# mrazomej/BarBay.jl

Measured on AMD Instinct MI355X. Metric: ELBO-grad steps/sec, 50k barcodes x 8 timepoints, higher is better.
Workload: dtype f64

## Files before the change

barbay.jl_amd/csrc/bb_engine.hip:

```cpp
#include "../../include/barbay_hip.h"
#include "bb_block.h"
#include "bb_persist.h"
#include "bb_resident.h"
#include "bb_stream.h"
#include "bb_inst.h"
#include "bb_hier.h"
#include "bb_ppc.h"
#include "bb_freq.h"
#include "bb_score.h"
#include "bb_rb.h"
#include "bb_chain.h"
#include "bb_trace.h"
#include "bb_logp.h"
#include "bb_mathprobe.h"

#include <algorithm>
#include <cmath>
#include <cstdarg>
#include <cstdio>
#include <cstdlib>
#include <cstring>
#include <ctime>
#include <string>
#include <type_traits>
// ... 228 lines not shown
            bbp_prefetch_slot<KIND, PP>(cx, h->M, h->S, A, h->NB, st + (size_t)b * h->nthr, bb_slot_of(A, step).slot);
            bbp_residual_ahead<KIND>(cx, h->M, h->NB, A);
            if (xg) bbp_consume<true>(cx, h->M, h->S, A, L, par, epoch, &E.ok, abs_epoch);
            else bbp_consume<false>(cx, h->M, h->S, A, L, par, epoch, &E.ok, abs_epoch);
            bbp_finish<KIND>(cx, h->M, h->S, A, h->NB);
            bbp_update<KIND, PP>(cx, h->M, h->S, A, h->NB, st + (size_t)b * h->nthr, bb_slot_of(A, step));
        }
    } else {
        for (int b = 0; b < h->nblk; ++b) {
            BBCtx cx = cxof(b);
            bbp_epilogue<KIND, PP>(cx, h->M, h->S, A, h->NB, st + (size_t)b * h->nthr, (unsigned long long)(h->step + nsteps), E.ok == 0);
        }
    }
}

template <int KIND, int PP, bool AP, bool OS = false>
static void emu_res_phase(EmuPersist& E, int phase, long long it, long long nsteps) {
    bb_handle* h = E.h;
    const RunArgs& A = E.A;
    BRSt<PP>* st = (BRSt<PP>*)E.st.data();
    auto cxof = [&](int b) { return BBCtx{h->nthr, b, E.lds.data() + (size_t)b * (h->lds_doubles_p + 64), nullptr}; };
    const BRLay& Y = h->Yh;
    const int NS = A.S < 1 ? 1 : A.S;
    const bool MSrun = NS > 1 || A.elbo_every > 0;
    const unsigned long long step = (unsigned long long)(h->step + it / NS);
    const int smp = (int)(it % NS);
    const bool last = smp == NS - 1;
    const unsigned long long xc = MSrun ? step * (unsigned long long)NS + (unsigned long long)smp : step;
    const int buf = (int)(xc & 1);
    const bool want_el = MSrun && A.elbo_every > 0 && step % (unsigned long long)A.elbo_every == 0;
    const int ring = A.elbo_every > 0 ? (int)((step / (unsigned long long)A.elbo_every) % BB_ELBO_RING) : 0;
    const bool xg = h->p2p_on;
    const BBSlot wslot = bb_slot_of(A, step);
    for (int b = 0; b < (phase == 2 ? bbp_groups(A) : h->plan.nblk); ++b) {
        BBCtx cx = cxof(b);
        BRSt<PP>* sb = st + (size_t)b * h->nthr;
        if (phase == 0) {
            br_prologue<KIND, PP, AP>(cx, h->M, h->S, A, Y, h->plan.NB, sb);
            br_draw_ahead<KIND, PP, AP>(cx, A, Y, sb, (unsigned long long)h->step);
        } else if (phase == 1) {
            if (MSrun) br_sample<KIND, PP, true>(cx, h->M, h->S, A, Y, sb, buf, wslot.slot, last, want_el);
            else br_sample<KIND, PP, false, false, OS>(cx, h->M, h->S, A, Y, sb, buf, wslot.slot);
            const unsigned epoch = A.xepoch0 + (unsigned)(xc + 1);
            if (MSrun) br_moments<KIND, PP, true>(cx, h->M, h->S, Y, sb, buf, epoch, want_el);
            else br_moments<KIND, PP, false>(cx, h->M, h->S, Y, sb, buf, epoch);
            br_xchg_publish<KIND, PP, AP, false, OS>(cx, h->M, h->S, A, Y, sb, xc, wslot.slot, last ? step + 1 : step, last ? 0u : (unsigned)(smp + 1), last);
        } else if (phase == 2) {
            if (xg) br_xchg_lead<true>(cx, h->M, h->S, A, Y, xc, &E.ok);
            else br_xchg_lead<false>(cx, h->M, h->S, A, Y, xc, &E.ok);
        } else if (phase == 3) {
            if (xg && MSrun) br_xchg_consume<KIND, PP, true, true>(cx, h->M, h->S, A, Y, sb, xc, &E.ok, want_el, ring, smp);
            else if (xg) br_xchg_consume<KIND, PP, true, false>(cx, h->M, h->S, A, Y, sb, xc, &E.ok);
            else if (MSrun) br_xchg_consume<KIND, PP, false, true>(cx, h->M, h->S, A, Y, sb, xc, &E.ok, want_el, ring, smp);
            else br_xchg_consume<KIND, PP, false, false>(cx, h->M, h->S, A, Y, sb, xc, &E.ok);
            if (MSrun) br_update<KIND, PP, 0, AP, true>(cx, h->M, h->S, A, Y, sb, wslot, buf, h->plan.NB, smp, NS);
            else if (!AP && uniform_T(h->M) == 8) br_update<KIND, PP, 8, false, false, false, OS>(cx, h->M, h->S, A, Y, sb, wslot, buf, h->plan.NB);
            else if (!AP && uniform_T(h->M) == 6) br_update<KIND, PP, 6, false, false, false, OS>(cx, h->M, h->S, A, Y, sb, wslot, buf, h->plan.NB);
            else br_update<KIND, PP, 0, AP, false, false, OS>(cx, h->M, h->S, A, Y, sb, wslot, buf, h->plan.NB);
        } else {
            br_epilogue<KIND, PP, AP>(cx, h->S, sb, (unsigned long long)(h->step + nsteps), E.ok == 0);
        }
    }
}

template <int KIND, int TT, bool MS, bool OS = false>
static void emu_stream_phase(EmuPersist& E, int phase, long long it, long long nsteps) {
    bb_handle* h = E.h;
    const RunArgs& A = E.A;
    BSG* gs = (BSG*)E.st.data();
    auto cxof = [&](int b) { return BBCtx{h->nthr, b, E.lds.data() + (size_t)b * (h->lds_doubles_p + 64), nullptr}; };
    const BRLay& Y = h->Yh;
    const int NS = MS ? (A.S < 1 ? 1 : A.S) : 1;
    const unsigned long long step = (unsigned long long)(h->step + it / NS);
    const int smp = (int)(it % NS);
    const unsigned long long xc = step * (unsigned long long)NS + (unsigned long long)smp;
    auto rec = [&](unsigned long long st_) { return MS && A.elbo_every > 0 && st_ % (unsigned long long)A.elbo_every == 0; };
    const bool want_el = rec(step);
    const int ring = A.elbo_every > 0 ? (int)((step / (unsigned long long)A.elbo_every) % BB_ELBO_RING) : 0;
    const BSMs ms = MS ? bs_ms_of(A, step, smp, NS, want_el, rec(step + 1)) : bs_ms_plain((unsigned)step);
    BRSt<1>* nost = nullptr;
    for (int b = 0; b < (phase == 2 ? bbp_groups(A) : h->plan.nblk); ++b) {
        BBCtx cx = cxof(b);
        BSG* gb = gs + (size_t)b * h->nthr;
        int* bad_any = (int*)(cx.lds + Y.L.misc) + 3;
        if (phase == 0) {
            br_tile_setup<KIND>(cx, h->M, h->S, A, Y, h->plan.NB, KIND <= 2 ? h->nthr / 16 : h->nthr / 64);
            *bad_any = 0;
            bs_sample0<KIND, TT, MS>(cx, h->M, h->S, A, Y, h->plan.NB, h->plan.P, (unsigned)h->step, gb, (int)(((unsigned long long)h->step * (unsigned long long)NS) & 1ull), rec((unsigned long long)h->step));
        } else if (phase == 1) {
            bs_moments<KIND, TT, MS>(cx, h->M, h->S, A, Y, h->plan.NB, h->plan.P, (unsigned)step, gb, ms.buf, want_el);
            br_row_publish<1, MS>(cx, h->M, h->S, Y, nost, A.xepoch0 + (unsigned)(xc + 1), want_el);
        } else if (phase == 2) {
            br_xchg_lead<false>(cx, h->M, h->S, A, Y, xc, &E.ok);
        } else if (phase == 3) {
            br_xchg_consume<KIND, 1, false, MS>(cx, h->M, h->S, A, Y, nost, xc, &E.ok, want_el, ring, smp);
            bs_update_l<KIND, TT, MS, OS>(cx, h->M, h->S, A, Y, h->plan.NB, h->plan.P, (unsigned)step, bb_slot_of(A, step), bad_any, gb, ms);
            bs_update_u<KIND, TT, MS, OS>(cx, h->M, h->S, A, Y, h->plan.NB, h->plan.P, (unsigned)step, bb_slot_of(A, step), bad_any, gb, ms);
        } else {
            if (*bad_any) h->S.hstatus[1] = 1u;
            if (b == 0) { h->S.ctr[0] = (unsigned long long)(h->step + nsteps); h->S.ctr[1] = h->S.ctr[0]; }
        }
    }
}

static void emu_persist_dispatch(EmuPersist& E, int phase, long long it, long long nsteps) {
    const LaunchPlan& p = E.h->plan;
// ... 621 lines not shown
```

barbay.jl_amd/csrc/bb_persist.h:

```cpp
#pragma once
#include "bb_block.h"
#include <string.h>

template <int KIND>
BB_DEV BBLds bbp_layout(const BBCtx& cx, const DevModel& M, int NB) {
    if (cx.lay) return *(const BBLds*)cx.lay;
    return bb_lds_layout(M.R, M.E, KIND, M.Ttot, M.nt1, M.K, NB, cx.nthr, 1);
}

template <int P>
struct BBPst {
    bb_d2 mu[P], om[P], am[P], ao[P];
    bb_d2 a[P], h[P];
    bb_d2 hm[P], ho[P];
    long long i0[P];
    int meta[P];
    bb_f4 lo[P];
};

#ifdef BB_EMU
#define BB_PSTATE(stv, tid) ((stv)[tid])
#else
#define BB_PSTATE(stv, tid) ((stv)[0])
#endif
// ... 260 lines not shown
    *word = v;
#else
    __hip_atomic_store(word, v, __ATOMIC_RELAXED, __HIP_MEMORY_SCOPE_AGENT);
#endif
}

BB_HD int bb_row_stride(int KK) { return KK; }
BB_DEV void bb_set_word64(unsigned long long* word, unsigned long long v) {
#ifdef BB_EMU
    *word = v;
#else
    __hip_atomic_store(word, v, __ATOMIC_RELAXED, __HIP_MEMORY_SCOPE_AGENT);
#endif
}
BB_DEV unsigned long long bb_get_word64(const unsigned long long* word) {
#ifdef BB_EMU
    return *word;
#else
    return __hip_atomic_load(word, __ATOMIC_RELAXED, __HIP_MEMORY_SCOPE_AGENT);
#endif
}
BB_DEV int br_xcc_id() {
#ifdef BB_EMU
    return 0;
#else
    return (int)(__builtin_amdgcn_s_getreg(20 | (0 << 6) | (3 << 11)) & 15u);
#endif
}

struct alignas(16) bb_gran { unsigned lo, t0, hi, t1; };
#ifndef BB_EMU
typedef unsigned bb_v4u __attribute__((ext_vector_type(4)));
#endif
template <bool SYS = false>
BB_DEV void bb_gran_st(bb_gran* p, double v, unsigned tag) {
#ifdef BB_EMU
    unsigned long long b;
    memcpy(&b, &v, 8);
    *p = bb_gran{(unsigned)b, tag, (unsigned)(b >> 32), tag};
#else
    bb_v4u g = {(unsigned)__double2loint(v), tag, (unsigned)__double2hiint(v), tag};
    if (SYS) asm volatile("global_store_dwordx4 %0, %1, off sc0 sc1" :: "v"(p), "v"(g) : "memory");
    else asm volatile("global_store_dwordx4 %0, %1, off sc1" :: "v"(p), "v"(g) : "memory");
#endif
}
BB_DEV void bb_gran_st_l2(bb_gran* p, double v, unsigned tag) {
#ifdef BB_EMU
    bb_gran_st(p, v, tag);
#else
    bb_v4u g = {(unsigned)__double2loint(v), tag, (unsigned)__double2hiint(v), tag};
    asm volatile("global_store_dwordx4 %0, %1, off" :: "v"(p), "v"(g) : "memory");
#endif
}
template <bool SYS = false>
BB_DEV bool bb_gran_poll8(const bb_gran* base, unsigned off, unsigned stride, int n, unsigned tag, bool active, unsigned* tmo, unsigned limit, double* out) {
#ifdef BB_EMU
    (void)tmo; (void)limit;
    bool good = true;
    for (int i = 0; i < 8; ++i) {
        out[i] = 0.0;
        if (!active || i >= n) continue;
        const bb_gran g = base[off + i * stride];
        good = good && g.t0 == tag && g.t1 == tag;
        const unsigned long long b = (unsigned long long)g.lo | ((unsigned long long)g.hi << 32);
        memcpy(&out[i], &b, 8);
    }
    return good;
#else
    bb_v4u g0, g1, g2, g3, g4, g5, g6, g7;
    bool ok = true;
    const unsigned sb = (unsigned)__builtin_amdgcn_readfirstlane((int)(stride * 16u));
    const unsigned long long bp = (unsigned long long)base;
    const unsigned long long sbase = ((unsigned long long)(unsigned)__builtin_amdgcn_readfirstlane((int)(bp >> 32)) << 32) | (unsigned)__builtin_amdgcn_readfirstlane((int)bp);
    for (unsigned spins = 0;; ++spins) {
        unsigned vo = off * 16u;
#define BB_POLL8(SC) \
        asm volatile("global_load_dwordx4 %0, %8, %9 " SC "\n\t" "v_add_u32 %8, %10, %8\n\t" \
                     "global_load_dwordx4 %1, %8, %9 " SC "\n\t" "v_add_u32 %8, %10, %8\n\t" \
                     "global_load_dwordx4 %2, %8, %9 " SC "\n\t" "v_add_u32 %8, %10, %8\n\t" \
                     "global_load_dwordx4 %3, %8, %9 " SC "\n\t" "v_add_u32 %8, %10, %8\n\t" \
                     "global_load_dwordx4 %4, %8, %9 " SC "\n\t" "v_add_u32 %8, %10, %8\n\t" \
                     "global_load_dwordx4 %5, %8, %9 " SC "\n\t" "v_add_u32 %8, %10, %8\n\t" \
                     "global_load_dwordx4 %6, %8, %9 " SC "\n\t" "v_add_u32 %8, %10, %8\n\t" \
                     "global_load_dwordx4 %7, %8, %9 " SC "\n\t" \
                     "s_waitcnt vmcnt(0)" \
                     : "=&v"(g0), "=&v"(g1), "=&v"(g2), "=&v"(g3), "=&v"(g4), "=&v"(g5), "=&v"(g6), "=&v"(g7), "+v"(vo) \
                     : "s"(sbase), "s"(sb) : "memory")
        if (SYS) BB_POLL8("sc0 sc1"); else BB_POLL8("sc1");
#undef BB_POLL8
        const bool good = ((g0.y == tag && g0.w == tag) || n < 1) && ((g1.y == tag && g1.w == tag) || n < 2) && ((g2.y == tag && g2.w == tag) || n < 3) &&
                          ((g3.y == tag && g3.w == tag) || n < 4) && ((g4.y == tag && g4.w == tag) || n < 5) && ((g5.y == tag && g5.w == tag) || n < 6) &&
                          ((g6.y == tag && g6.w == tag) || n < 7) && ((g7.y == tag && g7.w == tag) || n < 8);
        if (__builtin_amdgcn_ballot_w64(active && !good) == 0ull) break;
        __builtin_amdgcn_s_sleep(1);
        if ((spins & 255u) == 255u) {
            if (__hip_atomic_load(tmo, __ATOMIC_RELAXED, __HIP_MEMORY_SCOPE_AGENT) != 0u || spins > limit) {
                __hip_atomic_store(tmo, 1u, __ATOMIC_RELAXED, __HIP_MEMORY_SCOPE_AGENT);
                ok = false;
                break;
            }
        }
    }
#define BB_GV(g) __hiloint2double((int)g.z, (int)g.x)
    out[0] = n > 0 ? BB_GV(g0) : 0.0; out[1] = n > 1 ? BB_GV(g1) : 0.0; out[2] = n > 2 ? BB_GV(g2) : 0.0; out[3] = n > 3 ? BB_GV(g3) : 0.0;
    out[4] = n > 4 ? BB_GV(g4) : 0.0; out[5] = n > 5 ? BB_GV(g5) : 0.0; out[6] = n > 6 ? BB_GV(g6) : 0.0; out[7] = n > 7 ? BB_GV(g7) : 0.0;
#undef BB_GV
    return ok;
#endif
// ... 437 lines not shown
```

barbay.jl_amd/csrc/bb_plan.h:

```cpp

static int uniform_T(const DevModel& M) {
    for (int r = 1; r < M.R; ++r) if (M.T[r] != M.T[0]) return 0;
    return M.T[0];
}

static const void* resident_instance(const bb_handle* h, bool xg, bool stream, int P, bool ms, std::string& name, bool& os) {
    const int kind = h->M.kind, nthr = h->nthr, T = uniform_T(h->M);
    const bool ap = br_any_parity(h->M);
    const bool want_os = h->tune.opt_spec != 0 && !ms && h->o.optimizer == BB_OPT_TRUNCATED_ADAGRAD && h->o.resum_every == 0;
    os = false;
#if defined(BB_EMU)
    os = want_os;
    char nm[64];
    if (stream) snprintf(nm, sizeof nm, "emu:k_stream<%d,%d,%d%s>", kind, nthr, T, ms ? ",true" : "");
    else snprintf(nm, sizeof nm, "emu:k_res<%d,%d,%d,%s,*,%s,%s>", kind, P, nthr, xg ? "true" : "false", ap ? "true" : "false", ms ? "true" : "false");
    name = nm;
    return nullptr;
#elif defined(BB_FAST_BUILD)
    name = "(experiment build)";
    if (xg || ms) return nullptr;
    auto fn = [](auto k) { return (const void*)k; };
    if (stream) {
        if (nthr == 1024 && kind == 0 && T == 8) return fn(k_stream<0, 1024, 8>);
        if (nthr == 1024 && kind == 2 && T == 8) return fn(k_stream<2, 1024, 8>);
        if (nthr == 1024 && kind == 3 && T == 6) return fn(k_stream<3, 1024, 6>);
        return nullptr;
    }
    if (ap) {
        if (nthr > 512 && P == 1 && kind == 0) return fn(k_res<0, 1, 1024, false, 0, true>);
        if (nthr > 256 && nthr <= 512 && P == 3 && kind == 3) return fn(k_res<3, 3, 512, false, 0, true>);
        return nullptr;
    }
    if (nthr > 512 && P == 1 && kind == 0) return T == 8 ? fn(k_res<0, 1, 1024, false, 8>) : fn(k_res<0, 1, 1024, false>);
    if (nthr > 512 && P == 1 && kind == 1) return T == 6 ? fn(k_res<1, 1, 1024, false, 6>) : fn(k_res<1, 1, 1024, false>);
    if (nthr > 256 && nthr <= 512 && P == 2 && kind == 0) return T == 8 ? fn(k_res<0, 2, 512, false, 8>) : fn(k_res<0, 2, 512, false>);
    if (nthr > 256 && nthr <= 512 && P == 3 && kind == 3) return T == 6 ? fn(k_res<3, 3, 512, false, 6>) : fn(k_res<3, 3, 512, false>);
    if (nthr > 256 && nthr <= 512 && P == 2 && kind == 3) return T == 6 ? fn(k_res<3, 2, 512, false, 6>) : fn(k_res<3, 2, 512, false>);
    if (nthr > 512 && P == 1 && kind == 2) return T == 8 ? fn(k_res<2, 1, 1024, false, 8>) : fn(k_res<2, 1, 1024, false>);
    return nullptr;
#else
    const char* nm = "";
    const void* k = nullptr;
    if (want_os) k = stream ? (const void*)bb_stream_instance_os(kind, nthr, T, &nm) : (ap ? nullptr : (const void*)bb_res_instance_os(kind, P, nthr, xg, T, &nm));
    if (k) os = true;
    else if (stream) k = ms ? (const void*)bb_stream_instance_ms(kind, nthr, T, &nm) : (const void*)bb_stream_instance(kind, nthr, T, &nm);
    else switch (kind) {
        case 0: k = (const void*)bb_res_instance_k0(P, nthr, xg, T, ap, ms, &nm); break;
        case 1: k = (const void*)bb_res_instance_k1(P, nthr, xg, T, ap, ms, &nm); break;
        case 2: k = (const void*)bb_res_instance_k2(P, nthr, xg, T, ap, ms, &nm); break;
        case 3: k = (const void*)bb_res_instance_k3(P, nthr, xg, T, ap, ms, &nm); break;
        default: k = (const void*)bb_res_instance_k4(P, nthr, xg, T, ap, ms, &nm);
    }
    name = nm;
    return k;
#endif
}
static const void* persist_instance(const bb_handle* h, bool xg, int P, std::string& name) {
#if defined(BB_EMU)
    char nm[48];
    snprintf(nm, sizeof nm, "emu:k_persist<%d,%d,%d>", h->M.kind, P, h->nthr);
    name = nm;
    return nullptr;
#elif defined(BB_FAST_BUILD)
    name = "(experiment build)";
    if (!xg && h->nthr > 512 && P == 1 && h->M.kind == 0) return (const void*)k_persist<0, 1, 1024>;
    return nullptr;
#else
    const char* nm = "";
    const void* k = (const void*)bb_persist_instance(h->M.kind, P, h->nthr, xg, &nm);
    name = nm;
    return k;
#endif
}

static long long tile_pairs_bound(const DevModel& M, long long NB) {
    long long p = 0;
    for (int r = 0; r < M.R; ++r) p += NB * M.T[r] / 2 + 1;
    if (M.kind == 0 || M.kind == 1) p += 2 * (NB * M.E / 2 + 1);
    else if (M.kind == 2) p += 3 * (NB / 2 + 1);
    else if (M.kind == 3) p += (NB / 2 + 1) + 3ll * M.R * (NB / 2 + 1);
    else p += (NB * M.E / 2 + 1) + 3ll * M.R * (NB * M.E / 2 + 1);
    p += 2 * (M.nt1 / 2 + 1);
    return p;
}
// ... 98 lines not shown
    }
    if (tb.empty()) { tb.push_back(h->b_lo); tg.push_back(h->g_lo); }
    tb.push_back(h->b_hi);
    tg.push_back(h->g_hi);
    for (size_t i = 0; i + 1 < tg.size(); ++i) if (tg[i + 1] - tg[i] > NB) return false;
    return NB < 32768;
}

static bool geno_tile_table(const bb_handle* h, Planned& c) {
    const bool nb_fixed = h->tune.nb_set || h->tune.res_nb > 0;
    if (h->M.kind != BB_MODEL_GENOTYPE) return true;
    const int limit = std::max(c.nblk0, std::min(c.nblk0 + 8, h->cus));
    const int NB = c.plan.NB, NBL = c.plan.NBL, ng = c.plan.ng;
    bool ok = false;
    for (int grow = 0; grow <= NB / 2 + 8 && !ok; ++grow) {
        const int nb = NB + grow, nbl = NBL > 0 ? std::max(1, (int)((long long)NBL * nb / NB)) : 0;
        if (build_geno_tiles(h, nb, nbl, ng, c.tb, c.tg) && (int)c.tb.size() - 1 <= limit) { ok = true; c.plan.NB = nb; c.plan.NBL = nbl; }
        else if (nb_fixed && NBL > 0 && build_geno_tiles(h, nb, 0, ng, c.tb, c.tg) && (int)c.tb.size() - 1 <= limit) { ok = true; c.plan.NB = nb; c.plan.NBL = 0; }
    }
    if (!ok) return false;
    c.plan.nblk = (int)c.tb.size() - 1;
    return !(c.xg && c.plan.nblk < 8);
}

static bool pair_slots(const bb_handle* h, Planned& c) {
    const bool force_stream = h->tune.force_stream, no_stream = h->tune.no_stream;
    if (!c.xg && h->M.Dh != h->M.Dp) return false;
    c.plan.P = (int)((br_tile_span(h->M, c.plan.NB, true) + h->nthr - 1) / h->nthr);
    c.plan.impl = IMPL_RES;
    const int Pmax = h->nthr > 512 ? 2 : (h->nthr > 256 ? 3 : 4);
    if (!force_stream && c.plan.P <= Pmax) return true;
    const int T0 = uniform_T(h->M);
    const int Ps = (int)((br_tile_span(h->M, c.plan.NB, true, true) + h->nthr - 1) / h->nthr);
    if (!no_stream && !br_any_parity(h->M) && (T0 == 8 || T0 == 6 || T0 == 4) && h->nthr % 64 == 0 && !c.xg && Ps <= 64) {
        c.plan.impl = IMPL_STREAM;
        c.plan.P = Ps;
        c.scratch = h->o.samples_per_step > 1;
        return true;
    }
    return c.plan.P <= Pmax;
}

static bool window_fetch_layout(const bb_handle* h, Planned& c) {
    const bool stream = c.plan.impl == IMPL_STREAM;
    const int xrows = c.xg ? 8 * h->o.world_size : 0;
    c.plan.pf = h->o.optimizer == BB_OPT_TRUNCATED_ADAGRAD && !stream ? 1 : 0;
    c.Y = br_layout(h->M, c.plan.NB, h->nthr, c.plan.P, xrows, c.plan.pf == 1, stream);
    if (c.plan.pf != 0 && (size_t)c.Y.total * 8 > 160 * 1024) { c.plan.pf = 0; c.Y = br_layout(h->M, c.plan.NB, h->nthr, c.plan.P, xrows, false); }
    c.lds_doubles = (size_t)c.Y.total;
    return c.lds_doubles * 8 <= 160 * 1024;
}

static bool instance_fits(const bb_handle* h, Planned& c) {
    c.plan.fn = resident_instance(h, c.xg, c.plan.impl == IMPL_STREAM, c.plan.P, c.plan.ms, c.plan.name, c.plan.os);
    if (resident_fit(c.plan.fn, h->nthr, c.lds_doubles * 8, c.plan.nblk, h->cus)) return false;
    return c.plan.nblk <= h->tile_cap;
}

template <int KIND>
static void host_tables_kind(const bb_handle* h, const RunArgs& A, const DevState& Sh, Planned& c) {
    for (int b = 0; b < A.nblk; ++b) {
        const BBTile t = KIND == 2 ? br_tile_geno(h->M, Sh, b, c.plan.NB) : br_tile(h->M, A, b, c.plan.NB);
        const int g0 = KIND == 2 ? Sh.tile_g[b] : 0, g1 = KIND == 2 ? Sh.tile_g[b + 1] : 0;
        double* rec = c.segtab.data() + (size_t)b * c.segtab_stride;
        const int n = br_build_segs<KIND>((BRSeg*)rec, h->M, c.Y, t, b == 0, g0, g1);
        ((int*)(rec + c.segtab_stride - 1))[0] = n;
    }
}
static void host_tables(const bb_handle* h, Planned& c) {
    const bool off = h->tune.no_host_tables;
    if (off) return;
    const DevModel& M = h->M;
    c.segtab_stride = BR_SEG_DOUBLES * (4 + 4 * M.R + 1) + 1;
    RunArgs A = make_args(h, 0, 0, 1, true, false);
    A.nblk = c.plan.nblk; A.nbl = c.plan.NBL; A.ng = c.plan.ng;
    DevState Sh = h->S;
    Sh.tile_b = c.tb.data();
    Sh.tile_g = c.tg.data();
    c.segtab.assign((size_t)c.plan.nblk * c.segtab_stride, 0.0);
    by_kind(M.kind, [&](auto kindc) { host_tables_kind<decltype(kindc)::value>(h, A, Sh, c); });
    const int K = M.K, Tt = M.Ttot, R = M.R;
    c.ldstab.assign((size_t)3 * K + 4 * Tt + 4 * R + 4, 0);
    for (int j = 0; j < K; ++j) br_table_row(M, c.Y, j, &c.ldstab[2 * j], &c.ldstab[2 * K + j]);
    for (int j = 0; j < Tt; ++j) br_table_time(M, c.Y.L, j, &c.ldstab[3 * K + 4 * j]);
    for (int r = 0; r < R; ++r) br_table_rep(M, c.Y, r, &c.ldstab[3 * K + 4 * Tt + 4 * r]);
}

static bool plan_resident(const bb_handle* h, bool xg, bool any_parity, Planned& out) {
    const bool no_res = h->tune.no_res;
    if (no_res || !br_eligible(h->M) || (!any_parity && br_any_parity(h->M))) return false;
    Planned c;
    c.plan = two_kernel_plan(h);
    c.xg = xg;
    base_tile_map(h, c);
    if (!first_hop_groups(h, c)) return false;
    leader_tiles(h, c);
    if (!geno_tile_table(h, c) || !pair_slots(h, c) || !window_fetch_layout(h, c) || !instance_fits(h, c)) return false;
    host_tables(h, c);
    out = std::move(c);
    return true;
}

static const char* plan_persist(const bb_handle* h, bool xg, Planned& out) {
    Planned c;
    c.plan = two_kernel_plan(h);
    c.xg = xg;
    if (c.plan.ms) return h->o.samples_per_step != 1 ? "samples_per_step != 1 and the shape has no owner-computes instance" : "ELBO recording is on and the shape has no owner-computes instance";
// ... 73 lines not shown
```

barbay.jl_amd/csrc/bb_resident.h:

```cpp
#pragma once
#include "bb_persist.h"

#define BR_NCV 12
#if defined(BB_EMU) || defined(BR_NO_FENCE)
#define BR_SCHED_FENCE() ((void)0)
#else
#define BR_SCHED_FENCE() __builtin_amdgcn_sched_barrier(0)
#endif
#define BR_MAXT 16

struct BRSeg { long long lo, hi; int tbeg, span, blk, kind, ldsoff, r, lpb, T; double pm, iv; const double* mean_e; const double* iv_e; long long blo; int rstride, pad; };
#define BR_SEG_DOUBLES 12

struct BRLay {
    BBLds L;
    int zl, NBT;
    int zr0[BB_MAX_REP];
    int zlw, stw;
    int st[6], SU, nst;
    int eps;
    int hbuf;
    int racc;
    int racc_r[BB_MAX_REP], rw[BB_MAX_REP];
    int rowmap;
// ... 787 lines not shown
    }
}

template <int KIND, bool MS = false>
BB_DEV void br_finish(BBCtx& cx, const DevModel& M, const DevState& S, const BRLay& Y, const RunArgs* Ap = nullptr, bool want_el = false, int ring = 0, int smp = 0) {
    double* lds = cx.lds;
    const BBLds& L = Y.L;
    BB_STAMP(cx, S, 25);
    BB_STAMP_RT(cx, S, 30);
    BB_PASS(cx, tid) {
        for (int j = tid; j < M.Ttot; j += cx.nthr) {
            const int* ft = (const int*)(lds + Y.ftab) + 4 * j;
            const int mo = ft[0], zo = ft[1], hasprev = ft[2];
            double Dt = 0.0, c = 0.0, wb = 0.0;
            if (mo >= 0) {
                const double nn = (double)M.nn;
                const double* mm = lds + mo;
                const double M0 = mm[0], M1 = mm[1], N1 = mm[3], N2 = mm[4];
                const double sbar = lds[L.zgl + zo], ls = lds[L.zgl + M.nt1 + zo];
                wb = bb_exp(-2.0 * ls);
                const double dl = bb_log(lds[ft[3] + 1] * lds[L.invS + j]);
                const double cp = (dl - lds[Y.piv + j]) - sbar;
                c = dl - sbar;
                const double quadN = N2 - 2.0 * cp * N1 + nn * cp * cp;
                Dt = (M1 - cp * M0) + wb * (N1 - cp * nn);
                lds[L.gglob + zo] = -Dt;
                lds[L.gglob + M.nt1 + zo] = wb * quadN - nn;
                if (MS && want_el) {
                    const double M2 = mm[2], quadM = M2 - 2.0 * cp * M1 + cp * cp * M0;
                    lds[L.elbt + j] = -0.5 * (quadM + wb * quadN) - nn * ls;
                }
            } else if (MS && want_el) lds[L.elbt + j] = 0.0;
            lds[L.cc + j] = c;
            lds[L.wbar + j] = wb;
            lds[L.Dt + j] = Dt;
            lds[Y.iG + j] = ((hasprev ? lds[L.Dt + j - 1] : 0.0) - Dt) * lds[L.invS + j];
        }
    }
    BB_SYNC(cx);
    BB_STAMP(cx, S, 26);
    if (MS && want_el && cx.block == 0) {
        BB_PASS(cx, tid) {
            if (tid == 0) {
                const RunArgs& A = *Ap;
                double v = lds[L.wk + M.K - 2] + lds[L.wk + M.K - 1] + A.elbo_const;
                for (int j = 0; j < M.Ttot; ++j) v += lds[L.elbt + j];
                double* slot = S.elbo_ring + ring;
                *slot = (smp == 0 ? 0.0 : *slot) + v / (double)A.S;
            }
        }
    }
}

template <int KIND, int P>
BB_DEV void br_pair_prior(const double* lds, const BRLay& Y, const BRSt<P>& st, int k, bool a0, bool a1, double* pm0, double* iv0, double* pm1, double* iv1) {
    const BRSeg* sgk = (const BRSeg*)(lds + Y.seg) + (st.meta[k] >> 12);
    *pm0 = *pm1 = sgk->pm;
    *iv0 = *iv1 = sgk->iv;
    if (sgk->mean_e) {
        const long long j = st.i0[k] - sgk->blo;
        if (a0) { *pm0 = sgk->mean_e[j]; *iv0 = sgk->iv_e[j]; }
        if (a1) { *pm1 = sgk->mean_e[j + 1]; *iv1 = sgk->iv_e[j + 1]; }
    }
}
template <int KIND, int P>
BB_DEV void br_pair_diffs(const double* lds, const BRLay& Y, const BRSt<P>& st, int k, int buf, double* z0, double* z1,
                          double* ap, double* am, double* an, double* wp, double* wm, double* wn) {
    const int meta = st.meta[k];
    const bool hp = meta & BRM_PREV, hn = meta & BRM_NEXT;
    const double* zb = lds + Y.zl + buf * Y.NBT + st.zoff[k];
    *z0 = zb[0]; *z1 = zb[1];
    const double zp = hp ? zb[-1] : *z0, zn = hn ? zb[2] : *z1;
    *ap = *z0 - zp; *am = *z1 - *z0; *an = zn - *z1;
    *wp = *wm = *wn = 0.0;
    if (meta & BRM_MUT) {
        double sp, sm, sn;
        br_unit_sw<KIND>(lds, Y, buf, st.uo[k][1], KIND >= 2 ? st.thoff[k] : 0, &sm, wm);
        if (KIND == 1 || KIND == 4) {
            br_unit_sw<KIND>(lds, Y, buf, st.uo[k][0], KIND >= 3 ? st.thoff[k] : 0, &sp, wp);
            br_unit_sw<KIND>(lds, Y, buf, st.uo[k][2], KIND >= 3 ? st.thoff[k] : 0, &sn, wn);
        } else { sp = sn = sm; *wp = *wn = *wm; }
        *ap -= sp; *am -= sm; *an -= sn;
    }
}
template <int KIND, int P> BB_DEV constexpr bool br_has_pre() { return P == 1 && KIND <= 1; }
template <int KIND, int P, bool AP = false>
BB_DEV void br_grad_pre(BBCtx& cx, const BRLay& Y, BRSt<P>* stv, int buf) {
    if (!br_has_pre<KIND, P>()) return;
    const double* lds = cx.lds;
    BB_PASS(cx, tid) {
        BRSt<P>& st = BB_PSTATE(stv, tid);
#pragma unroll
        for (int k = 0; k < P; ++k) {
            const int meta = st.meta[k];
            if ((meta & 15) != SK_L || !(meta & BRM_VALID)) continue;
            const bool hp = meta & BRM_PREV, hn = meta & BRM_NEXT;
            double pm0, iv0, pm1, iv1, z0, z1, ap, am, an, wp, wm, wn;
            br_pair_prior<KIND>(lds, Y, st, k, true, AP ? (st.meta[k] & BRM_A1) != 0 : true, &pm0, &iv0, &pm1, &iv1);
            br_pair_diffs<KIND>(lds, Y, st, k, buf, &z0, &z1, &ap, &am, &an, &wp, &wm, &wn);
            double A0 = ((double)st.cnt[k][0] - st.lam[k].x) - (z0 - pm0) * iv0;
            double A1 = ((double)st.cnt[k][1] - st.lam[k].y) - (z1 - pm1) * iv1;
            if (meta & BRM_MUT) {
                const double ma = (AP && !(meta & BRM_A1)) ? 0.0 : wm * am;
                A0 += ma - (hp ? wp * ap : 0.0);
                A1 += (hn ? wn * an : 0.0) - ma;
            }
// ... 243 lines not shown
                BR_SCHED_FENCE();
                bb_opt_apply<OSK, OSK>(M, S, A, wslot, 1, ih + 1, -go1, ho.y, &nho.y, &st.om[k].y, &st.ao[k].y, &st.lo[k].w);
                BR_SCHED_FENCE();
            }
            if (OS || hs_m) { br_store_pair_stream<AP>(hs_m, ih, a0, a1, nhm); br_store_pair_stream<AP>(hs_o, ih, a0, a1, nho); }
        }
    }
#ifndef BB_EMU
    __builtin_amdgcn_s_setprio(0);
#endif
    BB_STAMP_WAVE(cx, S, A, 3);
    BB_STAMP(cx, S, 28);
}

template <int KIND, int P, bool AP = false>
BB_DEV void br_epilogue(BBCtx& cx, const DevState& S, BRSt<P>* stv, unsigned long long step_end, bool timed_out) {
    BB_PASS(cx, tid) {
        BRSt<P>& st = BB_PSTATE(stv, tid);
        bool bad = false;
#pragma unroll
        for (int k = 0; k < P; ++k) {
            const int meta = st.meta[k];
            if (!(meta & BRM_VALID)) continue;
            const bool a0 = meta & BRM_A0, a1 = meta & BRM_A1;
            br_store_pair<AP>(S.mu, st.i0[k], a0, a1, st.mu[k]);
            br_store_pair<AP>(S.om, st.i0[k], a0, a1, st.om[k]);
            br_store_pair<AP>(S.acc_mu, st.i0[k], a0, a1, st.am[k]);
            br_store_pair<AP>(S.acc_om, st.i0[k], a0, a1, st.ao[k]);
            bb_store_lo(S, st.i0[k], a0, a1, st.lo[k]);
            const double chk = (a0 ? st.mu[k].x + st.om[k].x : 0.0) + (a1 ? st.mu[k].y + st.om[k].y : 0.0);
            bad = bad || !(chk - chk == 0.0);
        }
        if (bad) S.hstatus[1] = 1u;
        if (timed_out && tid == 0) S.hstatus[0] = 1u;
        if (cx.block == 0 && tid == 0) { S.ctr[0] = step_end; S.ctr[1] = step_end; }
    }
    BB_SYNC(cx);
}

template <int KIND, int P, bool AP = false, bool HD = false, bool OS = false>
BB_DEV void br_xchg_publish(BBCtx& cx, const DevModel& M, const DevState& S, const RunArgs& A, const BRLay& Y, BRSt<P>* stv, unsigned long long xc, int slot,
                            unsigned long long next_step, unsigned next_stream = 0u, bool prefetch = true) {
    if (A.pf == 0 && prefetch) br_prefetch_slot<P, HD, OS>(cx, M, S, A, Y, stv, slot);
    br_grad_pre<KIND, P, AP>(cx, Y, stv, (int)(xc & 1));
    br_theta_sum<KIND, P>(cx, M, Y, stv);
    if (KIND == 3) br_theta_pre<KIND, P, 0>(cx, M, Y, stv, (int)(xc & 1));
    br_draw_ahead<KIND, P, AP>(cx, A, Y, stv, next_step, next_stream);
}
template <bool XG>
BB_DEV void br_xchg_lead(BBCtx& cx, const DevModel& M, const DevState& S, const RunArgs& A, const BRLay& Y, unsigned long long xc, int* ok_slot) {
    const unsigned epoch = A.xepoch0 + (unsigned)(xc + 1);
    if (cx.block < bbp_groups(A)) bbp_leader_reduce_tg<XG>(cx, M, S, A, Y.L, (int)(xc & 1), epoch, ok_slot);
}
template <int KIND, int P, bool XG, bool MS = false>
BB_DEV void br_xchg_consume(BBCtx& cx, const DevModel& M, const DevState& S, const RunArgs& A, const BRLay& Y, BRSt<P>* stv,
                            unsigned long long xc, int* ok_slot, bool want_el = false, int ring = 0, int smp = 0) {
    const unsigned epoch = A.xepoch0 + (unsigned)(xc + 1);
    if (XG) bbp_consume_tgx(cx, M, S, A, Y.L, (int)(xc & 1), epoch, ok_slot);
    else bbp_consume_tg(cx, M, S, A, Y.L, (int)(xc & 1), epoch, ok_slot);
    br_finish<KIND, MS>(cx, M, S, Y, &A, want_el, ring, smp);
}

#ifndef BB_EMU
template <int KIND, int P, int NT, bool XG = false, int TT = 0, bool AP = false, bool MS = false, bool OS = false>
__global__ void __launch_bounds__(NT) k_res(const DevModel* __restrict__ Mp, const DevState* __restrict__ Sp, const BRLay* __restrict__ Yp,
                                            RunArgs A, int NB, int nsteps) {
    const DevModel& M = *Mp;
    const DevState& S = *Sp;
    const BRLay& Y = *Yp;
    extern __shared__ __attribute__((aligned(16))) double br_smem[];
    BBCtx cx{(int)blockDim.x, (int)blockIdx.x, br_smem, nullptr};
    BRSt<P> st;
    int* ok_slot = (int*)(br_smem + Yp->L.misc) + 1;
    const unsigned long long c0 = S.ctr[0], c1 = S.ctr[1];
    unsigned long long step0 = c0 > c1 ? c0 : c1;
    step0 = ((unsigned long long)(unsigned)__builtin_amdgcn_readfirstlane((int)(step0 >> 32)) << 32) | (unsigned)__builtin_amdgcn_readfirstlane((int)step0);
    BB_STAMP_RT(cx, S, 2);
    br_prologue<KIND, P, AP>(cx, M, S, A, Y, NB, &st);
    BB_STAMP_RT(cx, S, 3);
    const bool dead = *ok_slot == 0;
    int done = 0;
    if (!dead) {
        br_draw_ahead<KIND, P, AP>(cx, A, Y, &st, step0);
        BB_STAMP_RT(cx, S, 4);
        BBSlotCtr sc = bb_slot_init<OS>(A, step0);
        const int NS = MS ? A.S : 1;
        int ec = (MS && A.elbo_every > 0) ? bb_uniform((int)(step0 % (unsigned long long)A.elbo_every)) : 1;
        int ring = (MS && A.elbo_every > 0) ? bb_uniform((int)(((step0 + (unsigned long long)A.elbo_every - 1ull) / (unsigned long long)A.elbo_every) % BB_ELBO_RING)) : 0;
        for (; done < nsteps; ++done, bb_slot_next<OS>(A, sc)) {
            const unsigned long long step = step0 + (unsigned long long)done;
            const BBSlot wslot = bb_slot_now<OS>(A, sc);
            const bool want_el = MS && A.elbo_every > 0 && ec == 0;
            bool stop = false;
            for (int smp = 0; smp < NS; ++smp) {
                const unsigned long long xc = MS ? step * (unsigned long long)NS + (unsigned long long)smp : step;
                const int buf = (int)(xc & 1);
                const bool last = smp == NS - 1;
                if (P > 1 || KIND >= 2) {
#pragma unroll
                    for (int k = 0; k < P; ++k) asm volatile("" : "+v"(st.meta[k]));
                }
                br_sample<KIND, P, MS, XG, OS>(cx, M, S, A, Y, &st, buf, wslot.slot, last, want_el);
                br_moments<KIND, P, MS>(cx, M, S, Y, &st, buf, A.xepoch0 + (unsigned)(xc + 1), want_el);
                br_xchg_publish<KIND, P, AP, XG, OS>(cx, M, S, A, Y, &st, xc, wslot.slot, last ? step + 1 : step, last ? 0u : (unsigned)(smp + 1), last);
                br_xchg_lead<XG>(cx, M, S, A, Y, xc, ok_slot);
                br_xchg_consume<KIND, P, XG, MS>(cx, M, S, A, Y, &st, xc, ok_slot, want_el, ring, smp);
                if (*ok_slot == 0) { stop = true; break; }
                br_update<KIND, P, TT, AP, MS, XG, OS>(cx, M, S, A, Y, &st, wslot, buf, NB, smp, NS);
            }
            if (stop) break;
            if (MS && A.elbo_every > 0) {
                if (ec == 0) ring = ring + 1 == BB_ELBO_RING ? 0 : ring + 1;
                ec = ec + 1 == A.elbo_every ? 0 : ec + 1;
            }
        }
    }
    BB_STAMP_RT(cx, S, 5);
    asm volatile("s_waitcnt vmcnt(0)" ::: "memory");
    br_epilogue<KIND, P, AP>(cx, S, &st, step0 + (unsigned long long)done, dead || *ok_slot == 0);
    BB_STAMP_RT(cx, S, 6);
}
#endif
```

Before: 72640.

## Fuse exchange consume and finish into single-wave specialized path for fixed T

Adds a specialized consume-and-finish routine for single-replicate models with uniform T of 6 or 8 under the optimizer-specialized path. One wave polls the group partial sums (with a fixed-8 full-poll variant), reduces them, and computes the per-timepoint global gradient terms directly in LDS. This replaces the generic consume followed by br_finish. It also adds new k_res instances with OS=true that the planner selects when the shape matches, so the optimizer-specialized kernels are now used for these shapes. The specialization is restricted to R==1 and at most 8 groups, and it adds code paths that must match the generic finish exactly.

```diff
diff --git a/barbay.jl_amd/csrc/bb_engine.hip b/barbay.jl_amd/csrc/bb_engine.hip
--- a/barbay.jl_amd/csrc/bb_engine.hip
+++ b/barbay.jl_amd/csrc/bb_engine.hip
@@ -304,6 +304,8 @@
             if (xg && MSrun) br_xchg_consume<KIND, PP, true, true>(cx, h->M, h->S, A, Y, sb, xc, &E.ok, want_el, ring, smp);
             else if (xg) br_xchg_consume<KIND, PP, true, false>(cx, h->M, h->S, A, Y, sb, xc, &E.ok);
             else if (MSrun) br_xchg_consume<KIND, PP, false, true>(cx, h->M, h->S, A, Y, sb, xc, &E.ok, want_el, ring, smp);
+            else if (OS && !AP && KIND <= 2 && uniform_T(h->M) == 8) br_xchg_consume<KIND, PP, false, false, br_fin_T<KIND, PP, false, 8, AP, false, OS>()>(cx, h->M, h->S, A, Y, sb, xc, &E.ok);
+            else if (OS && !AP && KIND <= 2 && uniform_T(h->M) == 6) br_xchg_consume<KIND, PP, false, false, br_fin_T<KIND, PP, false, 6, AP, false, OS>()>(cx, h->M, h->S, A, Y, sb, xc, &E.ok);
             else br_xchg_consume<KIND, PP, false, false>(cx, h->M, h->S, A, Y, sb, xc, &E.ok);
             if (MSrun) br_update<KIND, PP, 0, AP, true>(cx, h->M, h->S, A, Y, sb, wslot, buf, h->plan.NB, smp, NS);
             else if (!AP && uniform_T(h->M) == 8) br_update<KIND, PP, 8, false, false, false, OS>(cx, h->M, h->S, A, Y, sb, wslot, buf, h->plan.NB);
diff --git a/barbay.jl_amd/csrc/bb_persist.h b/barbay.jl_amd/csrc/bb_persist.h
--- a/barbay.jl_amd/csrc/bb_persist.h
+++ b/barbay.jl_amd/csrc/bb_persist.h
@@ -336,8 +336,9 @@
     asm volatile("global_store_dwordx4 %0, %1, off" :: "v"(p), "v"(g) : "memory");
 #endif
 }
-template <bool SYS = false>
-BB_DEV bool bb_gran_poll8(const bb_gran* base, unsigned off, unsigned stride, int n, unsigned tag, bool active, unsigned* tmo, unsigned limit, double* out) {
+template <bool SYS = false, bool FULL = false>
+BB_DEV bool bb_gran_poll8(const bb_gran* base, unsigned off, unsigned stride, int n_, unsigned tag, bool active, unsigned* tmo, unsigned limit, double* out) {
+    const int n = FULL ? 8 : n_;
 #ifdef BB_EMU
     (void)tmo; (void)limit;
     bool good = true;
diff --git a/barbay.jl_amd/csrc/bb_plan.h b/barbay.jl_amd/csrc/bb_plan.h
--- a/barbay.jl_amd/csrc/bb_plan.h
+++ b/barbay.jl_amd/csrc/bb_plan.h
@@ -4,10 +4,15 @@
     return M.T[0];
 }
 
-static const void* resident_instance(const bb_handle* h, bool xg, bool stream, int P, bool ms, std::string& name, bool& os) {
+static bool fin_chain_shape(const bb_handle* h, bool xg, bool stream, int P) {
+    const int T = uniform_T(h->M);
+    return !stream && !xg && !br_any_parity(h->M) && h->M.kind <= 2 && P <= 2 && (T == 8 || T == 6);
+}
+static const void* resident_instance(const bb_handle* h, bool xg, bool stream, int P, bool ms, int ng, std::string& name, bool& os) {
     const int kind = h->M.kind, nthr = h->nthr, T = uniform_T(h->M);
     const bool ap = br_any_parity(h->M);
-    const bool want_os = h->tune.opt_spec != 0 && !ms && h->o.optimizer == BB_OPT_TRUNCATED_ADAGRAD && h->o.resum_every == 0;
+    const bool fin_ok = !fin_chain_shape(h, xg, stream, P) || (h->M.R == 1 && ng <= 8);
+    const bool want_os = h->tune.opt_spec != 0 && !ms && h->o.optimizer == BB_OPT_TRUNCATED_ADAGRAD && h->o.resum_every == 0 && fin_ok;
     os = false;
 #if defined(BB_EMU)
     os = want_os;
@@ -30,6 +35,13 @@
         if (nthr > 512 && P == 1 && kind == 0) return fn(k_res<0, 1, 1024, false, 0, true>);
         if (nthr > 256 && nthr <= 512 && P == 3 && kind == 3) return fn(k_res<3, 3, 512, false, 0, true>);
         return nullptr;
+    }
+    if (want_os && nthr > 512 && P == 1) {
+        os = true;
+        if (kind == 0 && T == 8) return fn(k_res<0, 1, 1024, false, 8, false, false, true>);
+        if (kind == 1 && T == 6) return fn(k_res<1, 1, 1024, false, 6, false, false, true>);
+        if (kind == 2 && T == 8) return fn(k_res<2, 1, 1024, false, 8, false, false, true>);
+        os = false;
     }
     if (nthr > 512 && P == 1 && kind == 0) return T == 8 ? fn(k_res<0, 1, 1024, false, 8>) : fn(k_res<0, 1, 1024, false>);
     if (nthr > 512 && P == 1 && kind == 1) return T == 6 ? fn(k_res<1, 1, 1024, false, 6>) : fn(k_res<1, 1, 1024, false>);
@@ -234,7 +246,7 @@
 }
 
 static bool instance_fits(const bb_handle* h, Planned& c) {
-    c.plan.fn = resident_instance(h, c.xg, c.plan.impl == IMPL_STREAM, c.plan.P, c.plan.ms, c.plan.name, c.plan.os);
+    c.plan.fn = resident_instance(h, c.xg, c.plan.impl == IMPL_STREAM, c.plan.P, c.plan.ms, c.plan.ng, c.plan.name, c.plan.os);
     if (resident_fit(c.plan.fn, h->nthr, c.lds_doubles * 8, c.plan.nblk, h->cus)) return false;
     return c.plan.nblk <= h->tile_cap;
 }
diff --git a/barbay.jl_amd/csrc/bb_resident.h b/barbay.jl_amd/csrc/bb_resident.h
--- a/barbay.jl_amd/csrc/bb_resident.h
+++ b/barbay.jl_amd/csrc/bb_resident.h
@@ -863,6 +863,67 @@
     }
 }
 
+template <int KIND, int TT>
+BB_DEV void br_consume_finish(BBCtx& cx, const DevModel& M, const DevState& S, const RunArgs& A, int par, unsigned epoch, int* ok) {
+    static_assert(KIND <= 2 && TT >= 2 && 8 * TT - 5 <= 64, "one replicate whose row and time points fit one wave");
+    constexpr int K = 6 * TT - 3, NT1 = TT - 1, KK = K + 2 * NT1;
+    constexpr BRHdr H = br_header(K, NT1, TT, 1);
+    double* lds = cx.lds;
+    const int NG = bbp_groups(A);
+    double nn = (double)M.nn;
+#ifndef BB_EMU
+    asm volatile("" : "+v"(nn));
+#endif
+    BB_PASS(cx, tid) {
+        if (tid < 64) {
+            const bool act = tid < KK;
+            const int k = act ? tid : KK - 1;
+            double v[8];
+            bool good;
+            if (NG == 8) good = bb_gran_poll8<false, true>(S.gxrow + (long long)par * NG * KK, (unsigned)k, (unsigned)KK, 8, epoch, act, S.gbar + 1, A.spin_limit, v);
+            else good = bb_gran_poll8(S.gxrow + (long long)par * NG * KK, (unsigned)k, (unsigned)KK, NG, epoch, act, S.gbar + 1, A.spin_limit, v);
+            if (!good) *ok = 0;
+            BB_STAMP(cx, S, 1);
+            double s = 0.0;
+#pragma unroll
+            for (int i = 0; i < 8; ++i) s += v[i];
+            if (act) {
+                if (k < K) {
+                    lds[H.wk + k] = s;
+                    if (k < TT) lds[H.invS + k] = bb_rcp(s);
+                } else lds[H.zgl + (k - K)] = s;
+            }
+        }
+    }
+    BB_STAMP(cx, S, 25);
+    BB_STAMP_RT(cx, S, 30);
+    BB_PASS(cx, tid) {
+        if (tid < TT) {
+            const int j = tid;
+            double Dt = 0.0, c = 0.0, wb = 0.0;
+            if (j < TT - 1) {
+                const double* mm = lds + (H.wk + TT + 5 * j);
+                const double M0 = mm[0], M1 = mm[1], N1 = mm[3], N2 = mm[4];
+                const double sbar = lds[H.zgl + j], ls = lds[H.zgl + NT1 + j];
+                wb = bb_exp(-2.0 * ls);
+                const double dl = bb_log(lds[H.wk + j + 1] * lds[H.invS + j]);
+                const double cp = (dl - lds[H.piv + j]) - sbar;
+                c = dl - sbar;
+                const double quadN = N2 - 2.0 * cp * N1 + nn * cp * cp;
+                Dt = (M1 - cp * M0) + wb * (N1 - cp * nn);
+                lds[H.gglob + j] = -Dt;
+                lds[H.gglob + NT1 + j] = wb * quadN - nn;
+            }
+            lds[H.cc + j] = c;
+            lds[H.wbar + j] = wb;
+            lds[H.Dt + j] = Dt;
+            lds[H.iG + j] = ((j > 0 ? lds[H.Dt + j - 1] : 0.0) - Dt) * lds[H.invS + j];
+        }
+    }
+    BB_SYNC(cx);
+    BB_STAMP(cx, S, 26);
+}
+
 template <int KIND, int P>
 BB_DEV void br_pair_prior(const double* lds, const BRLay& Y, const BRSt<P>& st, int k, bool a0, bool a1, double* pm0, double* iv0, double* pm1, double* iv1) {
     const BRSeg* sgk = (const BRSeg*)(lds + Y.seg) + (st.meta[k] >> 12);
@@ -1212,10 +1273,12 @@
     const unsigned epoch = A.xepoch0 + (unsigned)(xc + 1);
     if (cx.block < bbp_groups(A)) bbp_leader_reduce_tg<XG>(cx, M, S, A, Y.L, (int)(xc & 1), epoch, ok_slot);
 }
-template <int KIND, int P, bool XG, bool MS = false>
+template <int KIND, int P, bool XG, int TT, bool AP, bool MS, bool OS> static inline constexpr int br_fin_T() { return (OS && !XG && !MS && !AP && KIND <= 2 && P <= 2 && TT > 0) ? TT : 0; }
+template <int KIND, int P, bool XG, bool MS = false, int FT = 0>
 BB_DEV void br_xchg_consume(BBCtx& cx, const DevModel& M, const DevState& S, const RunArgs& A, const BRLay& Y, BRSt<P>* stv,
                             unsigned long long xc, int* ok_slot, bool want_el = false, int ring = 0, int smp = 0) {
     const unsigned epoch = A.xepoch0 + (unsigned)(xc + 1);
+    if constexpr (FT > 0 && !XG && !MS && KIND <= 2) { br_consume_finish<KIND, FT>(cx, M, S, A, (int)(xc & 1), epoch, ok_slot); return; }
     if (XG) bbp_consume_tgx(cx, M, S, A, Y.L, (int)(xc & 1), epoch, ok_slot);
     else bbp_consume_tg(cx, M, S, A, Y.L, (int)(xc & 1), epoch, ok_slot);
     br_finish<KIND, MS>(cx, M, S, Y, &A, want_el, ring, smp);
@@ -1264,7 +1327,7 @@
                 br_moments<KIND, P, MS>(cx, M, S, Y, &st, buf, A.xepoch0 + (unsigned)(xc + 1), want_el);
                 br_xchg_publish<KIND, P, AP, XG, OS>(cx, M, S, A, Y, &st, xc, wslot.slot, last ? step + 1 : step, last ? 0u : (unsigned)(smp + 1), last);
                 br_xchg_lead<XG>(cx, M, S, A, Y, xc, ok_slot);
-                br_xchg_consume<KIND, P, XG, MS>(cx, M, S, A, Y, &st, xc, ok_slot, want_el, ring, smp);
+                br_xchg_consume<KIND, P, XG, MS, br_fin_T<KIND, P, XG, TT, AP, MS, OS>()>(cx, M, S, A, Y, &st, xc, ok_slot, want_el, ring, smp);
                 if (*ok_slot == 0) { stop = true; break; }
                 br_update<KIND, P, TT, AP, MS, XG, OS>(cx, M, S, A, Y, &st, wslot, buf, NB, smp, NS);
             }
```

New measurement: 76310 (median of 6 runs). 1.05x the previous value.
